# SonyResearch/micro_diffusion

Hardware: NVIDIA H100
Metric: training images/sec (global batch 2048) (higher is better)
Workload: dtype bf16

## Files before the change

micro_diffusion_b200/csrc/gemm_wgmma.cu:

```cuda
#include "gemm_wgmma.cuh"

#include <stdio.h>
#include <stdlib.h>

#include <type_traits>

#include "ptx.cuh"
#include "tensormap.cuh"

namespace md {

constexpr int kBlockM = 128;
constexpr int kBlockK = 64;
constexpr int kWgK = 16;
constexpr int kThreads = 384;

template <int BLOCK_N>
struct GemmCfg {
  static constexpr int kStageBytesA = kBlockM * kBlockK * 2;
  static constexpr int kStageBytesB = BLOCK_N * kBlockK * 2;
  static constexpr int kStageBytes = kStageBytesA + kStageBytesB;
  static constexpr int kStages = (192 * 1024) / kStageBytes;
  static constexpr int kSmemBytes = kStages * kStageBytes + 1024  + 256 ;
};

__device__ __forceinline__ float gelu_erf_fast(float x) {
  const float z = fabsf(x) * 0.70710678118654752440f;
  const float t = __fdividef(1.0f, fmaf(0.3275911f, z, 1.0f));
  float poly = fmaf(1.061405429f, t, -1.453152027f);
  poly = fmaf(poly, t, 1.421413741f);
  poly = fmaf(poly, t, -0.284496736f);
  poly = fmaf(poly, t, 0.254829592f);
  const float e = 1.0f - poly * t * __expf(-z * z);
  return 0.5f * x * (1.0f + copysignf(e, x));
}
__device__ __forceinline__ float gelu_tanh_fast(float x) {
  const float u = 0.7978845608028654f * fmaf(0.044715f * x, x * x, x);
  const float e = __expf(2.0f * u);
  const float th = 1.0f - __fdividef(2.0f, e + 1.0f);
  return 0.5f * x * (1.0f + th);
}

__device__ __forceinline__ float gelu_erf_grad_fast(float x) {
  const float z = fabsf(x) * 0.70710678118654752440f;
  const float t = __fdividef(1.0f, fmaf(0.3275911f, z, 1.0f));
  float poly = fmaf(1.061405429f, t, -1.453152027f);
  poly = fmaf(poly, t, 1.421413741f);
  poly = fmaf(poly, t, -0.284496736f);
  poly = fmaf(poly, t, 0.254829592f);
  const float ez = __expf(-z * z);
  const float e = 1.0f - poly * t * ez;
  const float cdf = 0.5f * (1.0f + copysignf(e, x));
  return fmaf(x * 0.3989422804014327f, ez, cdf);
}
__device__ __forceinline__ float gelu_tanh_grad_fast(float x) {
  const float k0 = 0.7978845608028654f, k1 = 0.044715f;
  const float u = k0 * fmaf(k1 * x, x * x, x);
  const float e = __expf(2.0f * u);
  const float th = 1.0f - __fdividef(2.0f, e + 1.0f);
  return 0.5f * (1.0f + th) + 0.5f * x * (1.0f - th * th) * k0 * fmaf(3.0f * k1 * x, x, 1.0f);
}

template <bool kTanh> __device__ __forceinline__ float gelu_fast(float x) {
  if constexpr (kTanh) return gelu_tanh_fast(x);
  else return gelu_erf_fast(x);
}
template <bool kTanh> __device__ __forceinline__ float gelu_grad_fast(float x) {
  if constexpr (kTanh) return gelu_tanh_grad_fast(x);
  else return gelu_erf_grad_fast(x);
}

constexpr int kBand = 8;
__device__ __forceinline__ void decode_tile(int r, int m_blocks, int n_blocks, int& mb, int& nb) {
  const int per_band = kBand * m_blocks;
  const int band = r / per_band;
  const int bw = min(kBand, n_blocks - band * kBand);
  const int rr = r - band * per_band;
  mb = rr / bw;
  nb = band * kBand + rr % bw;
}

__device__ __forceinline__ uint32_t pack_bf16(float a, float b) {
  __nv_bfloat162 v = __floats2bfloat162_rn(a, b);
  return *reinterpret_cast<uint32_t*>(&v);
}

__device__ __forceinline__ void st_bf16_pair(__nv_bfloat16* dst, float a, float b, bool two, bool vec) {
  if (two && vec) {
    *reinterpret_cast<uint32_t*>(dst) = pack_bf16(a, b);
  } else {
    dst[0] = __float2bfloat16_rn(a);
    if (two) dst[1] = __float2bfloat16_rn(b);
  }
}
__device__ __forceinline__ void st_f32_pair(float* dst, float a, float b, bool two, bool vec) {
  if (two && vec) {
    *reinterpret_cast<float2*>(dst) = make_float2(a, b);
  } else {
    dst[0] = a;
    if (two) dst[1] = b;
  }
}
__device__ __forceinline__ void red_f32_pair(float* dst, float a, float b, bool two, bool vec) {
  if (two && vec) {
    atomicAdd(reinterpret_cast<float2*>(dst), make_float2(a, b));
  } else {
    atomicAdd(dst, a);
    if (two) atomicAdd(dst + 1, b);
  }
}
__device__ __forceinline__ float2 ld_f32_pair(const float* src, bool two, bool vec) {
  if (two && vec) return *reinterpret_cast<const float2*>(src);
  return make_float2(src[0], two ? src[1] : 0.f);
}
__device__ __forceinline__ float2 ld_bf16_pair(const __nv_bfloat16* src, bool two, bool vec) {
  if (two && vec) return __bfloat1622float2(*reinterpret_cast<const __nv_bfloat162*>(src));
  return make_float2(__bfloat162float(src[0]), two ? __bfloat162float(src[1]) : 0.f);
}

template <int BLOCK_N, bool kMN>
__device__ __forceinline__ void wgmma_k16(float (&acc)[BLOCK_N / 2], uint64_t da, uint64_t db, uint32_t accumulate) {
  if constexpr (BLOCK_N == 256) wgmma_m64n256k16<kMN ? 1 : 0, kMN ? 1 : 0>(acc, da, db, accumulate);
  else wgmma_m64n128k16<kMN ? 1 : 0, kMN ? 1 : 0>(acc, da, db, accumulate);
}

template <int BLOCK_N, bool kMN>
__global__ void __launch_bounds__(kThreads, 1)
gemm_wgmma_kernel(const __grid_constant__ CUtensorMap tmA, const __grid_constant__ CUtensorMap tmB, const GemmDev p) {
  using Cfg = GemmCfg<BLOCK_N>;
  extern __shared__ uint8_t smem_raw[];
  uint8_t* smem = reinterpret_cast<uint8_t*>((reinterpret_cast<uintptr_t>(smem_raw) + 1023) &
                                             ~static_cast<uintptr_t>(1023));
  uint64_t* full_bar = reinterpret_cast<uint64_t*>(smem + Cfg::kStages * Cfg::kStageBytes);
  uint64_t* empty_bar = full_bar + Cfg::kStages;

  const int wg = threadIdx.x >> 7;
  const int warp = threadIdx.x >> 5;
  const int lane = threadIdx.x & 31;

  if (threadIdx.x == 0) {
    tma_prefetch_desc(&tmA);
    tma_prefetch_desc(&tmB);
    for (int i = 0; i < Cfg::kStages; ++i) {
      mbar_init(&full_bar[i], 1);
      mbar_init(&empty_bar[i], 8);
    }
    mbar_fence_init();
  }
  __syncthreads();

  const int m_blocks = (p.M + kBlockM - 1) / kBlockM;
  const int n_blocks = (p.N + BLOCK_N - 1) / BLOCK_N;
  const int kb_total = (p.K + kBlockK - 1) / kBlockK;
  const int kb_per_split = (kb_total + p.splits - 1) / p.splits;
  const long long mn = 1LL * n_blocks * m_blocks;
  const long long tiles = 1LL * p.batch * p.splits * mn;

  if (wg == 0) {
    warpgroup_reg_dealloc<40>();
    if (threadIdx.x == 0) {
      uint32_t it = 0;
      for (long long tile = blockIdx.x; tile < tiles; tile += gridDim.x) {
        long long t = tile;
        int mb, nb;
        decode_tile(static_cast<int>(t % mn), m_blocks, n_blocks, mb, nb);
        t /= mn;
        const int sp = t % p.splits; t /= p.splits;
        const int bz = static_cast<int>(t);
        const int kb0 = sp * kb_per_split;
        const int kb1 = min(kb_total, kb0 + kb_per_split);
        for (int kb = kb0; kb < kb1; ++kb, ++it) {
          const int s = it % Cfg::kStages;
          const uint32_t ph = (it / Cfg::kStages) & 1;
          mbar_wait(&empty_bar[s], ph ^ 1);
          uint8_t* sa = smem + s * Cfg::kStageBytes;
          uint8_t* sb = sa + Cfg::kStageBytesA;
          mbar_expect_tx(&full_bar[s], Cfg::kStageBytes);
          if constexpr (!kMN) {
            tma_load_3d(&tmA, &full_bar[s], sa, kb * kBlockK, mb * kBlockM, bz);
            tma_load_3d(&tmB, &full_bar[s], sb, kb * kBlockK, nb * BLOCK_N, bz);
          } else {
#pragma unroll
            for (int j = 0; j < kBlockM / 64; ++j)
              tma_load_3d(&tmA, &full_bar[s], sa + j * (kBlockK * 128), mb * kBlockM + j * 64, kb * kBlockK, bz);
#pragma unroll
            for (int j = 0; j < BLOCK_N / 64; ++j)
              tma_load_3d(&tmB, &full_bar[s], sb + j * (kBlockK * 128), nb * BLOCK_N + j * 64, kb * kBlockK, bz);
          }
        }
      }
    }
    return;
  }

  warpgroup_reg_alloc<232>();
  const int half = wg - 1;
  const int wq = warp & 3;
  constexpr uint32_t lbo = kMN ? (kBlockK * 128) : 16;
  constexpr uint32_t sbo = 1024;
  constexpr uint32_t kstep = (kMN ? (kWgK * 128) : (kWgK * 2)) >> 4;
  float acc[BLOCK_N / 2];
#pragma unroll
  for (int i = 0; i < BLOCK_N / 2; ++i) acc[i] = 0.f;
  const bool vec = p.vec2 != 0;
  const float alpha = p.alpha;

  uint32_t it = 0;
  for (long long tile = blockIdx.x; tile < tiles; tile += gridDim.x) {
    long long t = tile;
    int mb, nb;
    decode_tile(static_cast<int>(t % mn), m_blocks, n_blocks, mb, nb);
    t /= mn;
    const int sp = t % p.splits; t /= p.splits;
    const int bz = static_cast<int>(t);
    const int kb0 = sp * kb_per_split;
    const int kb1 = min(kb_total, kb0 + kb_per_split);
    const bool has_k = kb0 < kb_total;

    for (int kb = kb0; kb < kb1; ++kb, ++it) {
      const int s = it % Cfg::kStages;
      mbar_wait(&full_bar[s], (it / Cfg::kStages) & 1);
      const uint32_t sa = smem_u32(smem + s * Cfg::kStageBytes) + half * (64 * 128);
      const uint32_t sb = smem_u32(smem + s * Cfg::kStageBytes + Cfg::kStageBytesA);
      const uint64_t da0 = wgmma_smem_desc(sa, lbo, sbo);
      const uint64_t db0 = wgmma_smem_desc(sb, lbo, sbo);
      wgmma_fence();
#pragma unroll
      for (int k = 0; k < kBlockK / kWgK; ++k)
        wgmma_k16<BLOCK_N, kMN>(acc, da0 + k * kstep, db0 + k * kstep, (kb > kb0 || k > 0) ? 1u : 0u);
      wgmma_commit();
      wgmma_wait<1>();
      if (kb > kb0) {
        __syncwarp();
        if (lane == 0) mbar_arrive(&empty_bar[(it - 1) % Cfg::kStages]);
      }
    }
    wgmma_wait<0>();
    wgmma_fence_operands(acc);
    if (kb1 > kb0) {
      __syncwarp();
      if (lane == 0) mbar_arrive(&empty_bar[(it - 1) % Cfg::kStages]);
    }

    const int r0 = mb * kBlockM + half * 64 + wq * 16 + (lane >> 2);
    const int cb = nb * BLOCK_N + 2 * (lane & 3);
    auto for_each_pair = [&](auto&& f) {
#pragma unroll
      for (int i = 0; i < 2; ++i) {
        const int row = r0 + 8 * i;
        if (row >= p.M) continue;
        int row_out = row;
        if (p.row_interleave > 0) {
          const int blk = row >> 6, in = row & 63;
          row_out = (in < 32 ? 0 : p.row_interleave) + 32 * blk + (in & 31);
        }
        const long long crow = 1LL * bz * p.strideC + 1LL * row_out * p.ldc;
#pragma unroll
        for (int j = 0; j < BLOCK_N / 8; ++j) {
          const int col = cb + 8 * j;
          if (col < p.N) f(row, crow, i, j, col, acc[4 * j + 2 * i] * alpha, acc[4 * j + 2 * i + 1] * alpha, col + 1 < p.N);
        }
      }
    };
    auto add_bias = [&](int col, float& v0, float& v1, bool two) {
      if (p.bias != nullptr) {
        const float* b = p.bias + 1LL * bz * p.strideBias + col;
        v0 += b[0];
        if (two) v1 += b[1];
      }
    };

    switch (p.epi) {
      case EPI_STORE_BF16:
        for_each_pair([&](int, long long crow, int, int, int col, float v0, float v1, bool two) {
          add_bias(col, v0, v1, two);
          st_bf16_pair(reinterpret_cast<__nv_bfloat16*>(p.C) + crow + col, v0, v1, two, vec);
        });
        break;
      case EPI_STORE_F32:
        for_each_pair([&](int, long long crow, int, int, int col, float v0, float v1, bool two) {
          add_bias(col, v0, v1, two);
          st_f32_pair(reinterpret_cast<float*>(p.C) + crow + col, v0, v1, two, vec);
        });
        break;
      case EPI_RESID_F32:
        for_each_pair([&](int row, long long crow, int, int, int col, float v0, float v1, bool two) {
          add_bias(col, v0, v1, two);
          if (p.C2 != nullptr) st_bf16_pair(reinterpret_cast<__nv_bfloat16*>(p.C2) + crow + col, v0, v1, two, vec);
          if (p.gate != nullptr) {
            const float2 g = ld_f32_pair(p.gate + 1LL * (row / p.rows_per_gate) * p.ldgate + col, two, vec);
            v0 *= g.x;
            v1 *= g.y;
          }
          const long long rrow = 1LL * bz * p.strideC + 1LL * (p.res_mod > 0 ? row % p.res_mod : row) * p.ldc;
          const float2 r = ld_f32_pair(p.res + rrow + col, two, vec);
          st_f32_pair(reinterpret_cast<float*>(p.C) + crow + col, v0 + r.x, v1 + r.y, two, vec);
        });
        break;
      case EPI_ATOMIC_F32:
        if (p.split_ws != nullptr) {
          for_each_pair([&](int row, long long, int, int, int col, float v0, float v1, bool two) {
            float* dst = p.split_ws + ((1LL * sp * p.batch + bz) * p.M + row) * p.N + col;
            st_f32_pair(dst, has_k ? v0 : 0.f, has_k ? v1 : 0.f, two, vec);
          });
        } else if (has_k) {
          for_each_pair([&](int, long long crow, int, int, int col, float v0, float v1, bool two) {
            add_bias(col, v0, v1, two);
            red_f32_pair(reinterpret_cast<float*>(p.C) + crow + col, v0, v1, two, vec);
          });
        }
        break;
      case EPI_ACT_DUAL: {
        auto dual = [&](auto tanh_tag) {
          constexpr bool kTanh = decltype(tanh_tag)::value;
          for_each_pair([&](int, long long crow, int, int, int col, float v0, float v1, bool two) {
            add_bias(col, v0, v1, two);
            const float x0 = bf16_round(v0), x1 = bf16_round(v1);
            st_bf16_pair(reinterpret_cast<__nv_bfloat16*>(p.C) + crow + col, x0, x1, two, vec);
            st_bf16_pair(reinterpret_cast<__nv_bfloat16*>(p.C2) + crow + col, gelu_fast<kTanh>(x0), gelu_fast<kTanh>(x1), two,
                         vec);
          });
        };
        if (p.act) dual(std::true_type{});
        else dual(std::false_type{});
        break;
      }
      case EPI_ACT_GRAD: {
        auto grad = [&](auto tanh_tag) {
          constexpr bool kTanh = decltype(tanh_tag)::value;
          for_each_pair([&](int, long long crow, int, int, int col, float v0, float v1, bool two) {
            const float2 x = ld_bf16_pair(reinterpret_cast<const __nv_bfloat16*>(p.aux) + crow + col, two, vec);
            st_bf16_pair(reinterpret_cast<__nv_bfloat16*>(p.C) + crow + col, v0 * gelu_grad_fast<kTanh>(x.x),
                         v1 * gelu_grad_fast<kTanh>(x.y), two, vec);
          });
        };
        if (p.act) grad(std::true_type{});
        else grad(std::false_type{});
        break;
      }
      case EPI_SWIGLU:
        for_each_pair([&](int row, long long crow, int i, int j, int col, float, float, bool) {
          if ((j & 7) >= 4) return;
          const float a0 = bf16_round(acc[4 * j + 2 * i] * alpha), a1 = bf16_round(acc[4 * j + 2 * i + 1] * alpha);
          const float b0 = bf16_round(acc[4 * (j + 4) + 2 * i] * alpha), b1 = bf16_round(acc[4 * (j + 4) + 2 * i + 1] * alpha);
          __nv_bfloat16* du = reinterpret_cast<__nv_bfloat16*>(p.C) + crow + col;
          st_bf16_pair(du, a0, a1, true, true);
          st_bf16_pair(du + 32, b0, b1, true, true);
          const float h0 = a0 * __fdividef(1.0f, 1.0f + __expf(-a0)) * b0;
          const float h1 = a1 * __fdividef(1.0f, 1.0f + __expf(-a1)) * b1;
          st_bf16_pair(reinterpret_cast<__nv_bfloat16*>(p.C2) + 1LL * bz * p.strideC2 + 1LL * row * p.ldc2 +
                           (col >> 6) * 32 + (col & 63),
                       h0, h1, true, true);
        });
        break;
      case EPI_SWIGLU_GRAD:
        for_each_pair([&](int, long long crow, int, int, int col, float d0, float d1, bool) {
          const long long off = crow + 64 * (col >> 5) + (col & 31);
          const float2 u1 = ld_bf16_pair(reinterpret_cast<const __nv_bfloat16*>(p.aux) + off, true, true);
          const float2 u2 = ld_bf16_pair(reinterpret_cast<const __nv_bfloat16*>(p.aux) + off + 32, true, true);
          const float s0 = __fdividef(1.0f, 1.0f + __expf(-u1.x)), s1 = __fdividef(1.0f, 1.0f + __expf(-u1.y));
          __nv_bfloat16* dst = reinterpret_cast<__nv_bfloat16*>(p.C) + off;
          st_bf16_pair(dst, d0 * u2.x * (s0 * fmaf(u1.x, 1.0f - s0, 1.0f)), d1 * u2.y * (s1 * fmaf(u1.y, 1.0f - s1, 1.0f)),
                       true, true);
          st_bf16_pair(dst + 32, d0 * u1.x * s0, d1 * u1.y * s1, true, true);
        });
        break;
      default:
        break;
    }
  }
}

__global__ void __launch_bounds__(256)
splitk_reduce_kernel(const float* __restrict__ ws, float* __restrict__ C, int splits, int batch, int M, int N,
                     long long ldc, long long strideC, int row_interleave) {
  const long long total = 1LL * batch * M * N;
  for (long long i = 1LL * blockIdx.x * blockDim.x + threadIdx.x; i < total; i += 1LL * gridDim.x * blockDim.x) {
    const int n = static_cast<int>(i % N);
    const long long bm = i / N;
    const int m = static_cast<int>(bm % M);
    const int b = static_cast<int>(bm / M);
    float s = 0.f;
    for (int sp = 0; sp < splits; ++sp) s += ws[1LL * sp * total + i];
    int row = m;
    if (row_interleave > 0) {
      const int blk = m >> 6, in = m & 63;
      row = (in < 32 ? 0 : row_interleave) + 32 * blk + (in & 31);
    }
    C[1LL * b * strideC + 1LL * row * ldc + n] += s;
  }
}


static int make_map(CUtensorMap* map, const void* ptr, long long cols, long long rows, long long batch,
                    long long ld, long long batch_stride, int box_rows) {
  if ((reinterpret_cast<uintptr_t>(ptr) & 15) != 0 || (ld % 8) != 0 || (batch > 1 && (batch_stride % 8) != 0))
    return md_set_error(MD_ERR_INVALID, "gemm operand must be 16-byte aligned with ld %% 8 == 0");
  const TmapKey key = make_tmap_key(ptr, cols, rows, batch, ld, batch > 1 ? batch_stride : rows * ld, 64, box_rows,
                                    CU_TENSOR_MAP_SWIZZLE_128B, CU_TENSOR_MAP_L2_PROMOTION_L2_256B);
  CUresult r = cached_tensor_map(map, key);
  if (r != CUDA_SUCCESS) {
    char msg[160];
    snprintf(msg, sizeof(msg), "cuTensorMapEncodeTiled failed (%d) cols=%lld rows=%lld ld=%lld", (int)r, cols,
             rows, ld);
    return md_set_error(MD_ERR_CUDA, msg);
  }
  return 0;
}

template <int BLOCK_N, bool kMN>
static int launch(const md_gemm_args* a, const GemmDev& dev, int sm_count, cudaStream_t stream) {
  using Cfg = GemmCfg<BLOCK_N>;
  CUtensorMap tmA, tmB;
  int rc;
  if (!kMN) {
    rc = make_map(&tmA, a->A, a->K, a->M, a->batch, a->lda, a->strideA, kBlockM);
    if (rc) return rc;
    rc = make_map(&tmB, a->B, a->K, a->N, a->batch, a->ldb, a->strideB, BLOCK_N);
    if (rc) return rc;
  } else {
    rc = make_map(&tmA, a->A, a->M, a->K, a->batch, a->lda, a->strideA, kBlockK);
    if (rc) return rc;
    rc = make_map(&tmB, a->B, a->N, a->K, a->batch, a->ldb, a->strideB, kBlockK);
    if (rc) return rc;
  }
  auto kern = gemm_wgmma_kernel<BLOCK_N, kMN>;
  static bool attr_set = false;
  if (!attr_set) {
    cudaError_t e = cudaFuncSetAttribute(kern, cudaFuncAttributeMaxDynamicSharedMemorySize, Cfg::kSmemBytes);
    if (e != cudaSuccess) return md_set_error(MD_ERR_CUDA, cudaGetErrorString(e));
    attr_set = true;
  }
  const long long m_blocks = (a->M + kBlockM - 1) / kBlockM;
  const long long n_blocks = (a->N + BLOCK_N - 1) / BLOCK_N;
  const long long tiles = a->batch * dev.splits * m_blocks * n_blocks;
  const int grid = static_cast<int>(tiles < sm_count ? tiles : sm_count);
  kern<<<grid, kThreads, Cfg::kSmemBytes, stream>>>(tmA, tmB, dev);
  return check_launch("md_gemm_bf16");
}

}

extern "C" int md_gemm_bf16(const md_gemm_args* a, void* stream_) {
  using namespace md;
  cudaStream_t stream = reinterpret_cast<cudaStream_t>(stream_);
  if (a == nullptr || a->A == nullptr || a->B == nullptr || a->C == nullptr)
    return md_set_error(MD_ERR_INVALID, "md_gemm_bf16: null operand");
  if (a->M <= 0 || a->N <= 0 || a->K <= 0 || a->batch <= 0) return 0;
  if (a->epilogue < 0 || a->epilogue >= EPI_COUNT) return md_set_error(MD_ERR_INVALID, "md_gemm_bf16: bad epilogue");
  if (a->epilogue == EPI_RESID_F32 && a->res == nullptr)
    return md_set_error(MD_ERR_INVALID, "md_gemm_bf16: residual epilogue needs res");
  if (a->epilogue == EPI_ACT_DUAL && a->C2 == nullptr)
    return md_set_error(MD_ERR_INVALID, "md_gemm_bf16: activation epilogue needs C2");
  if (a->epilogue == EPI_ACT_GRAD && a->aux == nullptr)
    return md_set_error(MD_ERR_INVALID, "md_gemm_bf16: activation-gradient epilogue needs aux (the saved pre-activation)");
  if (a->epilogue == EPI_ACT_GRAD && a->bias != nullptr)
    return md_set_error(MD_ERR_INVALID, "md_gemm_bf16: the activation-gradient epilogue takes no bias");
  if (a->epilogue == EPI_SWIGLU || a->epilogue == EPI_SWIGLU_GRAD) {
    const bool fwd = a->epilogue == EPI_SWIGLU;
    const void* second = fwd ? a->C2 : a->aux;
    const int64_t ld2 = fwd ? (a->ldc2 > 0 ? a->ldc2 : a->N / 2) : a->ldc;
    if (second == nullptr || a->bias != nullptr || a->layout != MD_GEMM_NT || a->splits > 1)
      return md_set_error(MD_ERR_INVALID, "md_gemm_bf16: SwiGLU epilogues need C2 (forward) / aux (backward), NT layout, no bias");
    if (a->N % (fwd ? 64 : 32) != 0 || (a->ldc % 16) != 0 || (ld2 % 16) != 0 ||
        ((reinterpret_cast<uintptr_t>(a->C) | reinterpret_cast<uintptr_t>(second)) & 31) != 0 ||
        (a->batch > 1 && ((a->strideC % 16) != 0 || (fwd && (a->strideC2 % 16) != 0))))
      return md_set_error(MD_ERR_UNSUPPORTED,
                          "md_gemm_bf16: SwiGLU epilogues need 32-byte aligned outputs, pitches % 16 == 0 and whole 32-column blocks");
  }
  if (a->row_interleave != 0 && (a->epilogue != EPI_ATOMIC_F32 || a->row_interleave % 32 != 0 || a->M != 2 * a->row_interleave))
    return md_set_error(MD_ERR_INVALID, "md_gemm_bf16: row_interleave = f needs the atomic epilogue, f % 32 == 0 and M == 2 f");
  if (a->gate != nullptr && a->rows_per_gate <= 0)
    return md_set_error(MD_ERR_INVALID, "md_gemm_bf16: gate needs rows_per_gate > 0");
  int splits = a->splits > 0 ? a->splits : 1;
  if (splits > 1 && a->epilogue != EPI_ATOMIC_F32)
    return md_set_error(MD_ERR_INVALID, "md_gemm_bf16: split-K needs the atomic epilogue");

  int dev_id = 0, sm_count = 0;
  cudaError_t e = cudaGetDevice(&dev_id);
  if (e != cudaSuccess) return md_set_error(MD_ERR_CUDA, cudaGetErrorString(e));
  static int cached_sm[64] = {0};
  if (dev_id < 64 && cached_sm[dev_id] > 0) sm_count = cached_sm[dev_id];
  else {
    int major = 0;
    cudaDeviceGetAttribute(&sm_count, cudaDevAttrMultiProcessorCount, dev_id);
    cudaDeviceGetAttribute(&major, cudaDevAttrComputeCapabilityMajor, dev_id);
    if (major != 9) return md_set_error(MD_ERR_UNSUPPORTED, "md_gemm_bf16: requires an sm_90a device (H100)");
    if (dev_id < 64) cached_sm[dev_id] = sm_count;
  }

  if (a->sm_limit > 0 && a->sm_limit < sm_count) sm_count = a->sm_limit;

  GemmDev dev;
  dev.C = a->C; dev.C2 = a->C2;
  dev.bias = reinterpret_cast<const float*>(a->bias);
  dev.res = reinterpret_cast<const float*>(a->res);
  dev.gate = reinterpret_cast<const float*>(a->gate);
  dev.aux = a->aux;
  dev.ldc2 = a->ldc2 > 0 ? a->ldc2 : a->N / 2;
  dev.strideC2 = a->strideC2;
  dev.row_interleave = static_cast<int>(a->row_interleave);
  dev.split_ws = nullptr;
  dev.M = static_cast<int>(a->M); dev.N = static_cast<int>(a->N); dev.K = static_cast<int>(a->K);
  dev.batch = static_cast<int>(a->batch); dev.splits = splits;
  dev.ldc = a->ldc; dev.strideC = a->strideC; dev.strideBias = a->strideBias;
  dev.ldgate = a->ldgate; dev.rows_per_gate = static_cast<int>(a->rows_per_gate > 0 ? a->rows_per_gate : 1);
  dev.epi = a->epilogue;
  dev.res_mod = static_cast<int>(a->res_mod);
  dev.act = a->act;
  dev.alpha = a->alpha == 0.0f ? 1.0f : a->alpha;
  {
    const uintptr_t ptrs = reinterpret_cast<uintptr_t>(a->C) | reinterpret_cast<uintptr_t>(a->C2) |
                           reinterpret_cast<uintptr_t>(a->bias) | reinterpret_cast<uintptr_t>(a->res) |
                           reinterpret_cast<uintptr_t>(a->gate) | reinterpret_cast<uintptr_t>(a->aux);
    const long long pitches = a->N | a->ldc | a->strideC | dev.ldc2 | a->strideC2 | a->strideBias | a->ldgate;
    dev.vec2 = ((ptrs & 7) == 0 && (pitches & 1) == 0) ? 1 : 0;
  }

  const bool mn = a->layout == MD_GEMM_TN;
  const long long m_blocks = (a->M + kBlockM - 1) / kBlockM;
  const long long kb_total = (a->K + kBlockK - 1) / kBlockK;
  auto tiles_for = [&](int bn) { return a->batch * m_blocks * ((a->N + bn - 1) / bn); };
  const long long n256 = (a->N + 255) / 256 * 256;
  bool use256 = (a->N >= 256) && (n256 - a->N) * 5 <= a->N;
  if (a->splits == 0 && a->epilogue == EPI_ATOMIC_F32) {
    const long long t = tiles_for(use256 ? 256 : 128);
    const long long smax = kb_total / 8 > 0 ? (kb_total / 8 < 64 ? kb_total / 8 : 64) : 1;
    double best = 1e30;
    for (long long sp = 1; sp <= smax; ++sp) {
      const long long units = t * sp;
      const long long waves = (units + sm_count - 1) / sm_count;
      const double cost = static_cast<double>(waves) * (static_cast<double>((kb_total + sp - 1) / sp) + 10.0);
      if (cost < best - 1e-9) { best = cost; splits = static_cast<int>(sp); }
    }
    dev.splits = splits;
  } else if (use256 && tiles_for(256) * splits < sm_count && tiles_for(128) * splits > tiles_for(256) * splits) {
    use256 = false;
  }
  const bool math_tail = a->epilogue == EPI_SWIGLU || a->epilogue == EPI_SWIGLU_GRAD || a->epilogue == EPI_ACT_DUAL ||
                         a->epilogue == EPI_ACT_GRAD;
  if (math_tail && mn) return md_set_error(MD_ERR_UNSUPPORTED, "md_gemm_bf16: the activation / SwiGLU epilogues need the NT layout");
  if (det_enabled() && a->epilogue == EPI_ATOMIC_F32 && dev.splits > 1) {
    dev.split_ws = det_workspace(sizeof(float) * static_cast<size_t>(dev.splits) * a->batch * a->M * a->N);
    if (dev.split_ws == nullptr) dev.splits = 1;
  }
  auto run = [&]() -> int {
    if (mn) return use256 ? launch<256, true>(a, dev, sm_count, stream) : launch<128, true>(a, dev, sm_count, stream);
    return use256 ? launch<256, false>(a, dev, sm_count, stream) : launch<128, false>(a, dev, sm_count, stream);
  };
  if (int rc = run()) return rc;
  if (dev.split_ws != nullptr) {
    const long long total = 1LL * a->batch * a->M * a->N;
    const int blocks = static_cast<int>(total / 256 + 1 < 16LL * sm_count ? total / 256 + 1 : 16LL * sm_count);
    splitk_reduce_kernel<<<blocks, 256, 0, stream>>>(dev.split_ws, reinterpret_cast<float*>(a->C), dev.splits, dev.batch, dev.M,
                                                     dev.N, dev.ldc, dev.strideC, dev.row_interleave);
    return check_launch("md_gemm_bf16 (deterministic split-K reduction)");
  }
  return 0;
}
```

Baseline: 1121.

## Add ping-pong warpgroup schedule and batched epilogue loads to WGMMA GEMM

Adds a ping-pong variant in which each consumer warpgroup owns a whole 128x128 tile and alternates tiles with the other warpgroup. Ordering barriers hand the mainloop back and forth so one warpgroup's epilogue overlaps the other's MMAs. It is enabled for NT GEMMs with K<=1024, N<=4096 and store or SwiGLU epilogues, and forces BLOCK_N=128 there. Separately, the epilogues now issue bias, gate, residual and aux loads in chunks before the math, and use __ldg to hide load latency. The cost is more registers (128 accumulators per thread) and more mbarrier handoff overhead.

Result: faster. 1149, median of 6 (+2.5%).

```diff
diff --git a/micro_diffusion_b200/csrc/gemm_wgmma.cu b/micro_diffusion_b200/csrc/gemm_wgmma.cu
--- a/micro_diffusion_b200/csrc/gemm_wgmma.cu
+++ b/micro_diffusion_b200/csrc/gemm_wgmma.cu
@@ -117,6 +117,10 @@
   if (two && vec) return __bfloat1622float2(*reinterpret_cast<const __nv_bfloat162*>(src));
   return make_float2(__bfloat162float(src[0]), two ? __bfloat162float(src[1]) : 0.f);
 }
+__device__ __forceinline__ float2 ldg_f32_pair(const float* src, bool two, bool vec) {
+  if (two && vec) return __ldg(reinterpret_cast<const float2*>(src));
+  return make_float2(__ldg(src), two ? __ldg(src + 1) : 0.f);
+}
 
 template <int BLOCK_N, bool kMN>
 __device__ __forceinline__ void wgmma_k16(float (&acc)[BLOCK_N / 2], uint64_t da, uint64_t db, uint32_t accumulate) {
@@ -124,15 +128,17 @@
   else wgmma_m64n128k16<kMN ? 1 : 0, kMN ? 1 : 0>(acc, da, db, accumulate);
 }
 
-template <int BLOCK_N, bool kMN>
+template <int BLOCK_N, bool kMN, bool kPP>
 __global__ void __launch_bounds__(kThreads, 1)
 gemm_wgmma_kernel(const __grid_constant__ CUtensorMap tmA, const __grid_constant__ CUtensorMap tmB, const GemmDev p) {
+  static_assert(!kPP || BLOCK_N == 128, "ping-pong tiles are 128 x 128 (128 accumulator registers per thread)");
   using Cfg = GemmCfg<BLOCK_N>;
   extern __shared__ uint8_t smem_raw[];
   uint8_t* smem = reinterpret_cast<uint8_t*>((reinterpret_cast<uintptr_t>(smem_raw) + 1023) &
                                              ~static_cast<uintptr_t>(1023));
   uint64_t* full_bar = reinterpret_cast<uint64_t*>(smem + Cfg::kStages * Cfg::kStageBytes);
   uint64_t* empty_bar = full_bar + Cfg::kStages;
+  uint64_t* order_bar = empty_bar + Cfg::kStages;
 
   const int wg = threadIdx.x >> 7;
   const int warp = threadIdx.x >> 5;
@@ -143,8 +149,10 @@
     tma_prefetch_desc(&tmB);
     for (int i = 0; i < Cfg::kStages; ++i) {
       mbar_init(&full_bar[i], 1);
-      mbar_init(&empty_bar[i], 8);
-    }
+      mbar_init(&empty_bar[i], kPP ? 4 : 8);
+    }
+    mbar_init(&order_bar[0], 4);
+    mbar_init(&order_bar[1], 4);
     mbar_fence_init();
   }
   __syncthreads();
@@ -199,14 +207,19 @@
   constexpr uint32_t lbo = kMN ? (kBlockK * 128) : 16;
   constexpr uint32_t sbo = 1024;
   constexpr uint32_t kstep = (kMN ? (kWgK * 128) : (kWgK * 2)) >> 4;
-  float acc[BLOCK_N / 2];
-#pragma unroll
-  for (int i = 0; i < BLOCK_N / 2; ++i) acc[i] = 0.f;
+  constexpr int kSub = kPP ? 2 : 1;
+  float acc[kSub][BLOCK_N / 2];
+#pragma unroll
+  for (int s = 0; s < kSub; ++s)
+#pragma unroll
+    for (int i = 0; i < BLOCK_N / 2; ++i) acc[s][i] = 0.f;
   const bool vec = p.vec2 != 0;
   const float alpha = p.alpha;
 
   uint32_t it = 0;
-  for (long long tile = blockIdx.x; tile < tiles; tile += gridDim.x) {
+  uint32_t turn = 0;
+  int local = 0;
+  for (long long tile = blockIdx.x; tile < tiles; tile += gridDim.x, ++local) {
     long long t = tile;
     int mb, nb;
     decode_tile(static_cast<int>(t % mn), m_blocks, n_blocks, mb, nb);
@@ -216,18 +229,28 @@
     const int kb0 = sp * kb_per_split;
     const int kb1 = min(kb_total, kb0 + kb_per_split);
     const bool has_k = kb0 < kb_total;
+    if (kPP && (local & 1) != half) {
+      it += kb1 > kb0 ? kb1 - kb0 : 0;
+      continue;
+    }
+    if (kPP && local > 0) {
+      mbar_wait(&order_bar[half], turn & 1);
+      ++turn;
+    }
 
     for (int kb = kb0; kb < kb1; ++kb, ++it) {
       const int s = it % Cfg::kStages;
       mbar_wait(&full_bar[s], (it / Cfg::kStages) & 1);
-      const uint32_t sa = smem_u32(smem + s * Cfg::kStageBytes) + half * (64 * 128);
+      const uint32_t sa = smem_u32(smem + s * Cfg::kStageBytes) + (kPP ? 0 : half * (64 * 128));
       const uint32_t sb = smem_u32(smem + s * Cfg::kStageBytes + Cfg::kStageBytesA);
-      const uint64_t da0 = wgmma_smem_desc(sa, lbo, sbo);
       const uint64_t db0 = wgmma_smem_desc(sb, lbo, sbo);
       wgmma_fence();
 #pragma unroll
       for (int k = 0; k < kBlockK / kWgK; ++k)
-        wgmma_k16<BLOCK_N, kMN>(acc, da0 + k * kstep, db0 + k * kstep, (kb > kb0 || k > 0) ? 1u : 0u);
+#pragma unroll
+        for (int sub = 0; sub < kSub; ++sub)
+          wgmma_k16<BLOCK_N, kMN>(acc[sub], wgmma_smem_desc(sa + sub * (64 * 128), lbo, sbo) + k * kstep,
+                                  db0 + k * kstep, (kb > kb0 || k > 0) ? 1u : 0u);
       wgmma_commit();
       wgmma_wait<1>();
       if (kb > kb0) {
@@ -235,68 +258,129 @@
         if (lane == 0) mbar_arrive(&empty_bar[(it - 1) % Cfg::kStages]);
       }
     }
+    if (kPP && tile + gridDim.x < tiles) {
+      __syncwarp();
+      if (lane == 0) mbar_arrive(&order_bar[half ^ 1]);
+    }
     wgmma_wait<0>();
-    wgmma_fence_operands(acc);
+#pragma unroll
+    for (int sub = 0; sub < kSub; ++sub) wgmma_fence_operands(acc[sub]);
     if (kb1 > kb0) {
       __syncwarp();
       if (lane == 0) mbar_arrive(&empty_bar[(it - 1) % Cfg::kStages]);
     }
 
-    const int r0 = mb * kBlockM + half * 64 + wq * 16 + (lane >> 2);
+    const int r0 = mb * kBlockM + (kPP ? 0 : half * 64) + wq * 16 + (lane >> 2);
     const int cb = nb * BLOCK_N + 2 * (lane & 3);
+    constexpr int kGroups = 2 * kSub;
+    auto crow_of = [&](int row) {
+      int row_out = row;
+      if (p.row_interleave > 0) {
+        const int blk = row >> 6, in = row & 63;
+        row_out = (in < 32 ? 0 : p.row_interleave) + 32 * blk + (in & 31);
+      }
+      return 1LL * bz * p.strideC + 1LL * row_out * p.ldc;
+    };
     auto for_each_pair = [&](auto&& f) {
 #pragma unroll
-      for (int i = 0; i < 2; ++i) {
-        const int row = r0 + 8 * i;
+      for (int g = 0; g < kGroups; ++g) {
+        const int row = r0 + 64 * (g >> 1) + 8 * (g & 1);
         if (row >= p.M) continue;
-        int row_out = row;
-        if (p.row_interleave > 0) {
-          const int blk = row >> 6, in = row & 63;
-          row_out = (in < 32 ? 0 : p.row_interleave) + 32 * blk + (in & 31);
-        }
-        const long long crow = 1LL * bz * p.strideC + 1LL * row_out * p.ldc;
+        const long long crow = crow_of(row);
+        const float* a = acc[g >> 1];
+        const int i = g & 1;
 #pragma unroll
         for (int j = 0; j < BLOCK_N / 8; ++j) {
           const int col = cb + 8 * j;
-          if (col < p.N) f(row, crow, i, j, col, acc[4 * j + 2 * i] * alpha, acc[4 * j + 2 * i + 1] * alpha, col + 1 < p.N);
+          if (col < p.N) f(row, crow, g, j, col, a[4 * j + 2 * i] * alpha, a[4 * j + 2 * i + 1] * alpha, col + 1 < p.N);
         }
       }
     };
-    auto add_bias = [&](int col, float& v0, float& v1, bool two) {
-      if (p.bias != nullptr) {
-        const float* b = p.bias + 1LL * bz * p.strideBias + col;
-        v0 += b[0];
-        if (two) v1 += b[1];
+    auto for_each_pair_ld = [&](auto&& load, auto&& f) {
+      using Ld = decltype(load(0, 0LL, 0, true));
+      constexpr int kChunk = sizeof(Ld) <= 12 ? 8 : 4;
+#pragma unroll
+      for (int g = 0; g < kGroups; ++g) {
+        const int row = r0 + 64 * (g >> 1) + 8 * (g & 1);
+        if (row >= p.M) continue;
+        const long long crow = crow_of(row);
+        const float* a = acc[g >> 1];
+        const int i = g & 1;
+#pragma unroll
+        for (int j0 = 0; j0 < BLOCK_N / 8; j0 += kChunk) {
+          Ld ld[kChunk];
+#pragma unroll
+          for (int jj = 0; jj < kChunk; ++jj) {
+            const int col = cb + 8 * (j0 + jj);
+            if (col < p.N) ld[jj] = load(row, crow, col, col + 1 < p.N);
+          }
+#pragma unroll
+          for (int jj = 0; jj < kChunk; ++jj) {
+            const int j = j0 + jj, col = cb + 8 * j;
+            if (col < p.N)
+              f(row, crow, g, j, col, a[4 * j + 2 * i] * alpha, a[4 * j + 2 * i + 1] * alpha, col + 1 < p.N, ld[jj]);
+          }
+        }
+      }
+    };
+    const bool has_bias = p.bias != nullptr;
+    const float* bias_row = has_bias ? p.bias + 1LL * bz * p.strideBias : nullptr;
+    auto ld_bias = [&](int col, bool two) {
+      return has_bias ? ldg_f32_pair(bias_row + col, two, vec) : make_float2(0.f, 0.f);
+    };
+    auto add_bias = [&](float2 b, float& v0, float& v1, bool two) {
+      if (has_bias) {
+        v0 += b.x;
+        if (two) v1 += b.y;
+      }
+    };
+    auto ld_bias_only = [&](int, long long, int col, bool two) { return ld_bias(col, two); };
+    auto for_each_pair_bias = [&](auto&& f) {
+      if (has_bias) {
+        for_each_pair_ld(ld_bias_only, f);
+      } else {
+        for_each_pair([&](int row, long long crow, int g, int j, int col, float v0, float v1, bool two) {
+          f(row, crow, g, j, col, v0, v1, two, make_float2(0.f, 0.f));
+        });
       }
     };
 
     switch (p.epi) {
       case EPI_STORE_BF16:
-        for_each_pair([&](int, long long crow, int, int, int col, float v0, float v1, bool two) {
-          add_bias(col, v0, v1, two);
+        for_each_pair_bias([&](int, long long crow, int, int, int col, float v0, float v1, bool two, float2 b) {
+          add_bias(b, v0, v1, two);
           st_bf16_pair(reinterpret_cast<__nv_bfloat16*>(p.C) + crow + col, v0, v1, two, vec);
         });
         break;
       case EPI_STORE_F32:
-        for_each_pair([&](int, long long crow, int, int, int col, float v0, float v1, bool two) {
-          add_bias(col, v0, v1, two);
+        for_each_pair_bias([&](int, long long crow, int, int, int col, float v0, float v1, bool two, float2 b) {
+          add_bias(b, v0, v1, two);
           st_f32_pair(reinterpret_cast<float*>(p.C) + crow + col, v0, v1, two, vec);
         });
         break;
-      case EPI_RESID_F32:
-        for_each_pair([&](int row, long long crow, int, int, int col, float v0, float v1, bool two) {
-          add_bias(col, v0, v1, two);
-          if (p.C2 != nullptr) st_bf16_pair(reinterpret_cast<__nv_bfloat16*>(p.C2) + crow + col, v0, v1, two, vec);
-          if (p.gate != nullptr) {
-            const float2 g = ld_f32_pair(p.gate + 1LL * (row / p.rows_per_gate) * p.ldgate + col, two, vec);
-            v0 *= g.x;
-            v1 *= g.y;
-          }
-          const long long rrow = 1LL * bz * p.strideC + 1LL * (p.res_mod > 0 ? row % p.res_mod : row) * p.ldc;
-          const float2 r = ld_f32_pair(p.res + rrow + col, two, vec);
-          st_f32_pair(reinterpret_cast<float*>(p.C) + crow + col, v0 + r.x, v1 + r.y, two, vec);
-        });
-        break;
+      case EPI_RESID_F32: {
+        struct ResLd { float2 b, g, r; };
+        for_each_pair_ld(
+            [&](int row, long long, int col, bool two) {
+              ResLd l;
+              l.b = ld_bias(col, two);
+              l.g = p.gate != nullptr ? ldg_f32_pair(p.gate + 1LL * (row / p.rows_per_gate) * p.ldgate + col, two, vec)
+                                      : make_float2(1.f, 1.f);
+              const long long rrow = 1LL * bz * p.strideC + 1LL * (p.res_mod > 0 ? row % p.res_mod : row) * p.ldc;
+              l.r = ld_f32_pair(p.res + rrow + col, two, vec);
+              return l;
+            },
+            [&](int, long long crow, int, int, int col, float v0, float v1, bool two, ResLd l) {
+              add_bias(l.b, v0, v1, two);
+              if (p.C2 != nullptr) st_bf16_pair(reinterpret_cast<__nv_bfloat16*>(p.C2) + crow + col, v0, v1, two, vec);
+              if (p.gate != nullptr) {
+                v0 *= l.g.x;
+                v1 *= l.g.y;
+              }
+              st_f32_pair(reinterpret_cast<float*>(p.C) + crow + col, v0 + l.r.x, v1 + l.r.y, two, vec);
+            });
+        break;
+      }
       case EPI_ATOMIC_F32:
         if (p.split_ws != nullptr) {
           for_each_pair([&](int row, long long, int, int, int col, float v0, float v1, bool two) {
@@ -304,8 +388,8 @@
             st_f32_pair(dst, has_k ? v0 : 0.f, has_k ? v1 : 0.f, two, vec);
           });
         } else if (has_k) {
-          for_each_pair([&](int, long long crow, int, int, int col, float v0, float v1, bool two) {
-            add_bias(col, v0, v1, two);
+          for_each_pair_bias([&](int, long long crow, int, int, int col, float v0, float v1, bool two, float2 b) {
+            add_bias(b, v0, v1, two);
             red_f32_pair(reinterpret_cast<float*>(p.C) + crow + col, v0, v1, two, vec);
           });
         }
@@ -314,7 +398,10 @@
         auto dual = [&](auto tanh_tag) {
           constexpr bool kTanh = decltype(tanh_tag)::value;
           for_each_pair([&](int, long long crow, int, int, int col, float v0, float v1, bool two) {
-            add_bias(col, v0, v1, two);
+            if (has_bias) {
+              v0 += bias_row[col];
+              if (two) v1 += bias_row[col + 1];
+            }
             const float x0 = bf16_round(v0), x1 = bf16_round(v1);
             st_bf16_pair(reinterpret_cast<__nv_bfloat16*>(p.C) + crow + col, x0, x1, two, vec);
             st_bf16_pair(reinterpret_cast<__nv_bfloat16*>(p.C2) + crow + col, gelu_fast<kTanh>(x0), gelu_fast<kTanh>(x1), two,
@@ -339,10 +426,12 @@
         break;
       }
       case EPI_SWIGLU:
-        for_each_pair([&](int row, long long crow, int i, int j, int col, float, float, bool) {
+        for_each_pair([&](int row, long long crow, int g, int j, int col, float, float, bool) {
           if ((j & 7) >= 4) return;
-          const float a0 = bf16_round(acc[4 * j + 2 * i] * alpha), a1 = bf16_round(acc[4 * j + 2 * i + 1] * alpha);
-          const float b0 = bf16_round(acc[4 * (j + 4) + 2 * i] * alpha), b1 = bf16_round(acc[4 * (j + 4) + 2 * i + 1] * alpha);
+          const float* a = acc[g >> 1];
+          const int i = g & 1;
+          const float a0 = bf16_round(a[4 * j + 2 * i] * alpha), a1 = bf16_round(a[4 * j + 2 * i + 1] * alpha);
+          const float b0 = bf16_round(a[4 * (j + 4) + 2 * i] * alpha), b1 = bf16_round(a[4 * (j + 4) + 2 * i + 1] * alpha);
           __nv_bfloat16* du = reinterpret_cast<__nv_bfloat16*>(p.C) + crow + col;
           st_bf16_pair(du, a0, a1, true, true);
           st_bf16_pair(du + 32, b0, b1, true, true);
@@ -353,18 +442,26 @@
                        h0, h1, true, true);
         });
         break;
-      case EPI_SWIGLU_GRAD:
-        for_each_pair([&](int, long long crow, int, int, int col, float d0, float d1, bool) {
-          const long long off = crow + 64 * (col >> 5) + (col & 31);
-          const float2 u1 = ld_bf16_pair(reinterpret_cast<const __nv_bfloat16*>(p.aux) + off, true, true);
-          const float2 u2 = ld_bf16_pair(reinterpret_cast<const __nv_bfloat16*>(p.aux) + off + 32, true, true);
-          const float s0 = __fdividef(1.0f, 1.0f + __expf(-u1.x)), s1 = __fdividef(1.0f, 1.0f + __expf(-u1.y));
-          __nv_bfloat16* dst = reinterpret_cast<__nv_bfloat16*>(p.C) + off;
-          st_bf16_pair(dst, d0 * u2.x * (s0 * fmaf(u1.x, 1.0f - s0, 1.0f)), d1 * u2.y * (s1 * fmaf(u1.y, 1.0f - s1, 1.0f)),
-                       true, true);
-          st_bf16_pair(dst + 32, d0 * u1.x * s0, d1 * u1.y * s1, true, true);
-        });
-        break;
+      case EPI_SWIGLU_GRAD: {
+        struct U12 { __nv_bfloat162 u1, u2; };
+        for_each_pair_ld(
+            [&](int, long long crow, int col, bool) {
+              const __nv_bfloat162* src =
+                  reinterpret_cast<const __nv_bfloat162*>(reinterpret_cast<const __nv_bfloat16*>(p.aux) + crow + 64 * (col >> 5) +
+                                                          (col & 31));
+              return U12{src[0], src[16]};
+            },
+            [&](int, long long crow, int, int, int col, float d0, float d1, bool, U12 l) {
+              const long long off = crow + 64 * (col >> 5) + (col & 31);
+              const float2 u1 = __bfloat1622float2(l.u1), u2 = __bfloat1622float2(l.u2);
+              const float s0 = __fdividef(1.0f, 1.0f + __expf(-u1.x)), s1 = __fdividef(1.0f, 1.0f + __expf(-u1.y));
+              __nv_bfloat16* dst = reinterpret_cast<__nv_bfloat16*>(p.C) + off;
+              st_bf16_pair(dst, d0 * u2.x * (s0 * fmaf(u1.x, 1.0f - s0, 1.0f)), d1 * u2.y * (s1 * fmaf(u1.y, 1.0f - s1, 1.0f)),
+                           true, true);
+              st_bf16_pair(dst + 32, d0 * u1.x * s0, d1 * u1.y * s1, true, true);
+            });
+        break;
+      }
       default:
         break;
     }
@@ -408,7 +505,7 @@
   return 0;
 }
 
-template <int BLOCK_N, bool kMN>
+template <int BLOCK_N, bool kMN, bool kPP>
 static int launch(const md_gemm_args* a, const GemmDev& dev, int sm_count, cudaStream_t stream) {
   using Cfg = GemmCfg<BLOCK_N>;
   CUtensorMap tmA, tmB;
@@ -424,7 +521,7 @@
     rc = make_map(&tmB, a->B, a->N, a->K, a->batch, a->ldb, a->strideB, kBlockK);
     if (rc) return rc;
   }
-  auto kern = gemm_wgmma_kernel<BLOCK_N, kMN>;
+  auto kern = gemm_wgmma_kernel<BLOCK_N, kMN, kPP>;
   static bool attr_set = false;
   if (!attr_set) {
     cudaError_t e = cudaFuncSetAttribute(kern, cudaFuncAttributeMaxDynamicSharedMemorySize, Cfg::kSmemBytes);
@@ -523,6 +620,9 @@
   auto tiles_for = [&](int bn) { return a->batch * m_blocks * ((a->N + bn - 1) / bn); };
   const long long n256 = (a->N + 255) / 256 * 256;
   bool use256 = (a->N >= 256) && (n256 - a->N) * 5 <= a->N;
+  const bool pp = !mn && a->K <= 1024 && a->N <= 4096 &&
+                  (a->epilogue == EPI_STORE_BF16 || a->epilogue == EPI_STORE_F32 || a->epilogue == EPI_SWIGLU);
+  if (pp) use256 = false;
   if (a->splits == 0 && a->epilogue == EPI_ATOMIC_F32) {
     const long long t = tiles_for(use256 ? 256 : 128);
     const long long smax = kb_total / 8 > 0 ? (kb_total / 8 < 64 ? kb_total / 8 : 64) : 1;
@@ -545,8 +645,9 @@
     if (dev.split_ws == nullptr) dev.splits = 1;
   }
   auto run = [&]() -> int {
-    if (mn) return use256 ? launch<256, true>(a, dev, sm_count, stream) : launch<128, true>(a, dev, sm_count, stream);
-    return use256 ? launch<256, false>(a, dev, sm_count, stream) : launch<128, false>(a, dev, sm_count, stream);
+    if (mn) return use256 ? launch<256, true, false>(a, dev, sm_count, stream) : launch<128, true, false>(a, dev, sm_count, stream);
+    if (pp) return launch<128, false, true>(a, dev, sm_count, stream);
+    return use256 ? launch<256, false, false>(a, dev, sm_count, stream) : launch<128, false, false>(a, dev, sm_count, stream);
   };
   if (int rc = run()) return rc;
   if (dev.split_ws != nullptr) {
```
